# TuringQ/deepquantum

Measured on AMD Instinct MI355X. Metric: gate-applies/sec, 28q random circuit depth 40 (HBM GB/s in roofline), higher is better.
Workload: dtype c64

## Files before the change

### deepquantum_amd/csrc/dq_wave.hip

```cpp
#include <utility>

#include "dq_common.hpp"
#include <stddef.h>
#include <string.h>
#include <stdlib.h>

namespace dq {

#include "dq_wave_asm.inc"
#include "dq_wave_asm64.inc"
#include "dq_wave_valu.inc"
#include "dq_wave_valu64.inc"

constexpr int WAVE_LANES = 6;
constexpr int WAVE_MAX_REC = 112;
constexpr int WAVE_EXT_REC = 256;

struct WaveC64 {
    using real = float;
    using acc_t = float;
    static constexpr int M = 12, R = 6, NA = 64, VB = 1, MAXK = DQ_WAVE_MAXK, ELEM = 8, GRAD_VARIANTS = DQ_WAVE_GRAD_VARIANTS;
    static constexpr unsigned LDS_PER_WAVE = 8448;
    static constexpr int ID_GEN_U = DQ_WID_GEN_U, ID_GEN_C = DQ_WID_GEN_C, ID_GEN_R = DQ_WID_GEN_R, ID_X_U = DQ_WID_X_U,
                         ID_X_C = DQ_WID_X_C, ID_X_R = DQ_WID_X_R, ID_X_R1 = DQ_WID_X_R1, ID_TRIP0 = DQ_WID_TRIP0,
                         ID_DIAG1 = DQ_WID_DIAG1, ID_DIAG2 = DQ_WID_DIAG2, ID_GRAD = DQ_WID_GRAD, ID_EXPZ = DQ_WID_EXPZ, ID_GEN2 = DQ_WID_GEN2, ID_GEN2R = DQ_WID_GEN2R, ID_GEN2X = DQ_WID_GEN2X, ID_GEN2XC = DQ_WID_GEN2XC, ID_SWAP = DQ_WID_SWAP;
    static int trip_id(unsigned mask) { return kWaveTripId[mask]; }
    static int swap_id(int i, int j) { return kWaveSwapId[i][j]; }
    __device__ static __forceinline__ void body(uint64_t kg, uint32_t gend, uint64_t mb, uint32_t moff, uint64_t tg, uint64_t ks,
                                                uint64_t inb, uint64_t outb, uint32_t ldsb, uint32_t tid, uint32_t flags) {
        wave_tile_body_f32(kg, gend, mb, moff, tg, ks, inb, outb, ldsb, tid, flags);
    }
};
struct WaveC128 {
    using real = double;
    using acc_t = double;
    static constexpr int M = 11, R = 5, NA = 32, VB = 0, MAXK = DQ_WAVE64_MAXK, ELEM = 16, GRAD_VARIANTS = DQ_WAVE64_GRAD_VARIANTS;
    static constexpr unsigned LDS_PER_WAVE = 8704;
    static constexpr int ID_GEN_U = DQ_WID64_GEN_U, ID_GEN_C = DQ_WID64_GEN_C, ID_GEN_R = DQ_WID64_GEN_R, ID_X_U = DQ_WID64_X_U,
                         ID_X_C = DQ_WID64_X_C, ID_X_R = DQ_WID64_X_R, ID_X_R1 = DQ_WID64_X_R1, ID_TRIP0 = DQ_WID64_TRIP0,
                         ID_DIAG1 = DQ_WID64_DIAG1, ID_DIAG2 = DQ_WID64_DIAG2, ID_GRAD = DQ_WID64_GRAD, ID_EXPZ = DQ_WID64_EXPZ, ID_GEN2 = DQ_WID64_GEN2, ID_GEN2R = DQ_WID64_GEN2R, ID_GEN2X = -1, ID_GEN2XC = -1, ID_SWAP = DQ_WID64_SWAP;
    static int trip_id(unsigned mask) { return kWave64TripId[mask]; }
    static int swap_id(int i, int j) { return kWave64SwapId[i][j]; }
    __device__ static __forceinline__ void body(uint64_t kg, uint32_t gend, uint64_t mb, uint32_t moff, uint64_t tg, uint64_t ks,
                                                uint64_t inb, uint64_t outb, uint32_t ldsb, uint32_t tid, uint32_t flags) {
        wave_tile_body_f64(kg, gend, mb, moff, tg, ks, inb, outb, ldsb, tid, flags);
    }
};

template <typename T> using vec2 = T __attribute__((ext_vector_type(2)));

struct WaveRec {
    uint32_t w[8];
};

struct WaveKernPass {
    uint64_t load_off[5];
    uint64_t store_off[5];
    uint32_t load_lane_shift[6];
    uint32_t store_lane_shift[6];
    uint32_t tb_contrib[6];
    uint32_t nrec_bytes, mat_base_bytes;
    uint8_t read_blk_pos[DQ_FUSED_MAX_BLK];
    uint8_t store_blk_pos[DQ_FUSED_MAX_BLK];
    uint32_t zext;
    uint32_t fix_read[2], fix_write[2];
    uint32_t reserved[3];
    WaveRec rec[WAVE_MAX_REC];
};
static_assert(offsetof(WaveKernPass, store_off) == 40 && offsetof(WaveKernPass, load_lane_shift) == 80 &&
                  offsetof(WaveKernPass, tb_contrib) == 128 && offsetof(WaveKernPass, zext) == 208 &&
                  offsetof(WaveKernPass, rec) == 240, "descriptor layout");

struct WaveKernArgs {
    const void* in;
    void* out;
    const void* mats;
    int64_t mat_bstride;
    int64_t in_bstride;
    int n;
    int tpw;
    WaveKernPass p;
    double* grads;
    int64_t grad_bstride;
    const void* ext_rec;
};
static_assert(sizeof(WaveKernArgs) <= 4096 && (offsetof(WaveKernArgs, p) + offsetof(WaveKernPass, rec)) % 32 == 0, "kernel-argument segment");

template <class W, bool GRAD>
__global__ __launch_bounds__(256) void wave_pass_kernel(const vec2<typename W::real>* in, vec2<typename W::real>* out,
                                                        const vec2<typename W::real>* mats, int64_t mat_bstride,
                                                        int64_t in_bstride, int n, int tpw_flags, const WaveKernPass p,
                                                        double* grads, int64_t grad_bstride, const void* ext_rec) {
    (void)in, (void)out, (void)mats, (void)mat_bstride;
    extern __shared__ __attribute__((aligned(16))) unsigned char dq_wave_smem[];
    (void)dq_wave_smem;
    const unsigned tid = threadIdx.x;
    if constexpr (GRAD) {
        for (unsigned i = tid; i < p.nrec_bytes / 4u; i += 256u)
            *(__attribute__((address_space(3))) typename W::acc_t*)(uintptr_t)(4u * W::LDS_PER_WAVE + (unsigned)sizeof(typename W::acc_t) * i) = 0;
        __syncthreads();
    }
    const unsigned wave = (unsigned)__builtin_amdgcn_readfirstlane((int)(tid >> 6));
    unsigned grp = blockIdx.x, sample = blockIdx.y;
    if (in_bstride == 0 && (gridDim.x & 7u) == 0) {
        const unsigned lin = blockIdx.y * gridDim.x + blockIdx.x, nb = gridDim.y;
        const unsigned group = lin / (8u * nb), r = lin % (8u * nb);
        sample = r >> 3;
        grp = group * 8u + (r & 7u);
    }
    if (const unsigned xv = ((unsigned)tpw_flags >> 18) & 31u) {
        const unsigned q = blockIdx.x >> 3, j = blockIdx.x & 7u;
        if (xv == 31u) grp = j * (gridDim.x >> 3) + q;
        else grp = ((q >> (xv - 1u)) << (xv + 2u)) + (j << (xv - 1u)) + (q & ((1u << (xv - 1u)) - 1u));
    }
  uint32_t tile32 = grp * 4u + wave;
  for (;;) {
    const uint64_t tile_id = tile32;
    typedef const __attribute__((address_space(4))) uint32_t* KWords;
    uint64_t karg = (uint64_t)__builtin_amdgcn_kernarg_segment_ptr();
    asm volatile("" : "+s"(karg));
    const KWords hw = (KWords)(karg + offsetof(WaveKernArgs, p));
    {
        const uint32_t a_tf0 = ((KWords)karg)[offsetof(WaveKernArgs, tpw) / 4];
        const uint32_t ntiles = 1u << (hw[offsetof(WaveKernPass, zext) / 4] & 63u), lper = 2u + (a_tf0 & 0xffu);
        if (tile32 >= ntiles) break;
        tile32 += ((ntiles + (1u << lper) - 1u) >> lper) * 4u;
    }
    uint64_t tg = 0, tw = 0;
#pragma unroll
    for (int w = 0; w < DQ_FUSED_MAX_BLK / 4; ++w) {
        const uint32_t rw = hw[offsetof(WaveKernPass, read_blk_pos) / 4 + w], sw = hw[offsetof(WaveKernPass, store_blk_pos) / 4 + w];
#pragma unroll
        for (int k = 0; k < 4; ++k) {
            const uint64_t bit = (tile_id >> (4 * w + k)) & 1ull;
            tg |= bit << ((rw >> (8 * k)) & 0x3fu);
            tw |= bit << ((sw >> (8 * k)) & 0x3fu);
        }
    }
    {
        const uint32_t fo = offsetof(WaveKernPass, fix_read) / 4;
        tg |= (uint64_t)hw[fo] | ((uint64_t)hw[fo + 1] << 32);
        tw |= (uint64_t)hw[fo + 2] | ((uint64_t)hw[fo + 3] << 32);
    }
    typedef const __attribute__((address_space(4))) uint64_t* KQuads;
    const KQuads kq = (KQuads)karg;
    const uint64_t a_in = kq[0], a_out = kq[1], a_mats = kq[2], a_mbs = kq[3], a_ibs = kq[4];
    const uint64_t a_ext = kq[offsetof(WaveKernArgs, ext_rec) / 8];
    const uint64_t rec_base = a_ext ? a_ext : karg + offsetof(WaveKernArgs, p) + offsetof(WaveKernPass, rec);
    const uint32_t a_n = ((KWords)karg)[offsetof(WaveKernArgs, n) / 4], a_tf = ((KWords)karg)[offsetof(WaveKernArgs, tpw) / 4];
    constexpr uint64_t ES = W::ELEM;
    const uint64_t inb = a_in + ((uint64_t)sample * a_ibs + tg) * ES;
    const uint64_t outb = a_out + (((uint64_t)sample << a_n) + tw) * ES;
    const uint64_t mb = a_mats + (uint64_t)((int64_t)sample * (int64_t)a_mbs) * ES;
    const unsigned flags = ((a_ibs == 0 ? (a_tf >> 16) & ~1u : a_tf >> 16) & 3u) | (hw[offsetof(WaveKernPass, zext) / 4] & 0x003f3f00u);
    W::body(rec_base, hw[offsetof(WaveKernPass, nrec_bytes) / 4], mb,
            hw[offsetof(WaveKernPass, mat_base_bytes) / 4], tg,
            karg + offsetof(WaveKernArgs, p) + offsetof(WaveKernPass, load_off), inb, outb, wave * W::LDS_PER_WAVE, tid,
            flags);
  }
    if constexpr (GRAD) {
        __syncthreads();
        typedef const __attribute__((address_space(4))) uint32_t* KW;
        const KW rw = ext_rec ? (KW)(uint64_t)ext_rec
                              : (KW)((uint64_t)__builtin_amdgcn_kernarg_segment_ptr() + offsetof(WaveKernArgs, p) + offsetof(WaveKernPass, rec));
        const unsigned nrec = p.nrec_bytes / 32u;
        double* const grow = grads + (uint64_t)sample * (uint64_t)grad_bstride;
        for (unsigned i = tid; i < nrec * 8u; i += 256u) {
            const unsigned id = rw[8u * (i >> 3)];
            if ((id >= (unsigned)W::ID_GRAD && id < (unsigned)W::ID_EXPZ) || (id == (unsigned)W::ID_EXPZ && (i & 7u) == 0u)) {
                const typename W::acc_t v = *(__attribute__((address_space(3))) typename W::acc_t*)(uintptr_t)(4u * W::LDS_PER_WAVE + (unsigned)sizeof(typename W::acc_t) * i);
                atomicAdd(grow + (uint64_t)rw[8u * (i >> 3) + 6] * 8u + (i & 7u), (double)v);
            }
        }
    }
}

namespace {

template <class W>
struct Xlate {
    const DqFusedPass* p;
    WaveKernPass* k;
    int phys[W::R];
    int lanes[WAVE_LANES];
    int nrec = 0;
    WaveRec* recs = nullptr;
    int cap = WAVE_MAX_REC;

    bool push(const WaveRec& r) {
        if (nrec >= cap) return false;
        recs[nrec++] = r;
        return true;
    }
    int slot_of(int tile_bit) const {
        for (int s = 0; s < W::R; ++s)
            if (phys[s] == tile_bit) return s;
        return -1;
    }

    bool trip(unsigned mask, const int* inc_lanes, int kk, const int* want) {
        const int a = 5 - kk, S = 64 + (1 << a);
        int moving[W::R], out_bits[W::R], inc_bits[W::R], stay_lanes[WAVE_LANES], stay_bits[WAVE_LANES], fpos[WAVE_LANES];
        int nm = 0, ns = 0;
        for (int s = 0; s < W::R; ++s)
            if ((mask >> s) & 1u) {
                moving[nm] = s;
                out_bits[nm] = phys[s];
                ++nm;
            }
        for (int i = 0; i < kk; ++i) inc_bits[i] = lanes[inc_lanes[i]];
        for (int b = 0; b < WAVE_LANES; ++b) {
            bool inc = false;
            for (int i = 0; i < kk; ++i) inc = inc || inc_lanes[i] == b;
            if (!inc) {
                stay_lanes[ns] = b;
                stay_bits[ns] = lanes[b];
                ++ns;
            }
        }
        if (kk == 0) {
            for (int t = 0; t < ns; ++t) fpos[t] = t;
        } else {
            for (int t = 0; t < ns; ++t) fpos[t] = t < a ? t : 5;
        }
        uint32_t cw[WAVE_LANES] = {0}, cr[WAVE_LANES] = {0}, tbc[WAVE_LANES] = {0};
        for (int i = 0; i < kk; ++i) cw[inc_lanes[i]] = (unsigned)W::ELEM << (a + i);
        for (int t = 0; t < ns; ++t) cw[stay_lanes[t]] = (unsigned)W::ELEM << fpos[t];
        int nl[WAVE_LANES];
        if (want) {
            for (int b = 0; b < WAVE_LANES; ++b) nl[b] = want[b];
        } else if (kk == 0) {
            for (int b = 0; b < WAVE_LANES; ++b) nl[b] = lanes[b];
        } else {
            for (int b = 0; b < WAVE_LANES; ++b) nl[b] = b < a ? stay_bits[b] : (b < 5 ? out_bits[b - a] : stay_bits[a]);
        }
        for (int b = 0; b < WAVE_LANES; ++b) {
            bool found = false;
            for (int i = 0; i < kk && !found; ++i)
                if (nl[b] == out_bits[i]) {
                    cr[b] = ((unsigned)W::ELEM * (unsigned)S) << i;
                    found = true;
                }
            for (int t = 0; t < ns && !found; ++t)
                if (nl[b] == stay_bits[t]) {
                    cr[b] = (unsigned)W::ELEM << fpos[t];
                    found = true;
                }
            if (!found) return false;
            tbc[b] = 1u << nl[b];
        }
        WaveRec ra{}, rb{};
        ra.w[0] = kk == 0 ? (uint32_t)W::ID_TRIP0 : (uint32_t)W::trip_id(mask);
        ra.w[1] = tbc[0], ra.w[2] = tbc[1], ra.w[3] = tbc[2], ra.w[5] = tbc[3], ra.w[6] = tbc[4], ra.w[7] = tbc[5];
        for (int b = 0; b < WAVE_LANES; ++b) rb.w[b] = cw[b] | (cr[b] << 16);
        for (int i = 0; i < kk; ++i) phys[moving[i]] = inc_bits[i];
        for (int b = 0; b < WAVE_LANES; ++b) lanes[b] = nl[b];
        return push(ra) && push(rb);
    }

    bool go(unsigned slotset, const int* want) {
        for (;;) {
            unsigned mask = 0;
            int inc[WAVE_LANES], ninc = 0, nout = 0;
            for (int s = 0; s < W::R; ++s)
                if (!((slotset >> phys[s]) & 1u)) {
                    mask |= 1u << s;
                    ++nout;
                }
            for (int b = 0; b < WAVE_LANES; ++b)
                if ((slotset >> lanes[b]) & 1u) inc[ninc++] = b;
            if (nout != ninc) return false;
            if (nout == 0) return true;
            int kk = nout;
            if (kk > W::MAXK) kk = nout > 2 * W::MAXK ? W::MAXK : (nout + 1) / 2;
            if (kk < nout) {
                unsigned m2 = 0;
                int c = 0;
                for (int s = 0; s < W::R && c < kk; ++s)
                    if ((mask >> s) & 1u) {
                        m2 |= 1u << s;
                        ++c;
                    }
                mask = m2;
            }
            if (!trip(mask, inc, kk, kk == nout ? want : nullptr)) return false;
        }
    }
};

}

template <class W>
static int wave_translate(const DqFusedPass* p, int n, WaveKernPass* k, uint64_t dead = 0, WaveRec* ext = nullptr, int ext_cap = 0,
                          uint64_t fixm = 0, uint64_t fixv = 0) {
    memset(k, 0, sizeof(*k));
    const int L = p->L, h = p->h;
    auto rpos = [&](int tl) { return tl < L ? tl : (int)p->high_pos[tl - L]; };
    auto wpos = [&](int tl) { return tl < L ? (int)p->store_low_pos[tl] : (int)p->store_high_pos[tl - L]; };
    Xlate<W> x;
    x.p = p;
    x.k = k;
    x.recs = ext ? ext : k->rec;
    x.cap = ext ? ext_cap : WAVE_MAX_REC;
    unsigned slotmask = 0;
    for (int s = 0; s < W::R; ++s) {
        x.phys[s] = p->load_rb[s];
        slotmask |= 1u << p->load_rb[s];
    }
    for (int b = 0, q = 0; b < WAVE_LANES; ++b, ++q) {
        while ((slotmask >> q) & 1u) ++q;
        x.lanes[b] = q;
    }
    {
        uint64_t tilemask = (1ull << L) - 1ull;
        for (int i = 0; i < h; ++i) tilemask |= 1ull << p->high_pos[i];
        int nb = 0;
        uint64_t fix_r = 0, fix_w = 0;
        for (int j = 0, q = 0; j < n - W::M; ++j, ++q) {
            while (q < 64 && ((tilemask >> q) & 1ull)) ++q;
            if ((dead >> q) & 1ull) continue;
            if ((fixm >> q) & 1ull) {
                if ((fixv >> q) & 1ull) {
                    fix_r |= 1ull << q;
                    fix_w |= 1ull << p->store_blk_pos[j];
                }
                continue;
            }
            k->read_blk_pos[nb] = (uint8_t)q;
            k->store_blk_pos[nb] = p->store_blk_pos[j];
            ++nb;
        }
        for (int j = nb; j < DQ_FUSED_MAX_BLK; ++j) k->read_blk_pos[j] = k->store_blk_pos[j] = 63;
        k->zext = (uint32_t)nb;
        k->fix_read[0] = (uint32_t)fix_r, k->fix_read[1] = (uint32_t)(fix_r >> 32);
        k->fix_write[0] = (uint32_t)fix_w, k->fix_write[1] = (uint32_t)(fix_w >> 32);
        static const bool by_store = [] { const char* e = getenv("DQ_WAVE_TILE_ORDER"); return !(e && e[0] == 'r'); }();
        if (by_store)
            for (int i = 1; i < nb; ++i)
                for (int j = i; j > 0 && k->store_blk_pos[j] < k->store_blk_pos[j - 1]; --j) {
                    std::swap(k->store_blk_pos[j], k->store_blk_pos[j - 1]);
                    std::swap(k->read_blk_pos[j], k->read_blk_pos[j - 1]);
                }
    }
    for (int s = W::VB; s < W::R; ++s) {
        k->load_off[s - W::VB] = (uint64_t)W::ELEM << rpos(x.phys[s]);
        if ((dead >> rpos(x.phys[s])) & 1ull) k->zext |= 1u << (8 + s);
    }
    for (int b = 0; b < WAVE_LANES; ++b) {
        k->load_lane_shift[b] = (W::ELEM == 8 ? 3u : 4u) + (uint32_t)rpos(x.lanes[b]);
        k->tb_contrib[b] = 1u << x.lanes[b];
        if ((dead >> rpos(x.lanes[b])) & 1ull) k->zext |= 1u << (16 + b);
    }
    k->mat_base_bytes = p->mat_base * (uint32_t)W::ELEM;

    const char* why = "too many records for one pass (gates + layout changes)";
    for (int r = 0; r < p->nrounds; ++r) {
        const DqFusedRound& rd = p->rounds[r];
        unsigned want = 0;
        for (int s = 0; s < W::R; ++s) want |= 1u << rd.rb[s];
        if (!x.go(want, nullptr)) goto fail;
        for (int gi = rd.gate_begin; gi < rd.gate_end; ++gi) {
            const DqFusedGate& g = p->gates[gi];
            if (g.kind == DQ_FG_GEN2 && W::ID_GEN2 >= 0) {
                const int q1 = x.slot_of(rd.rb[g.q]), q2 = x.slot_of(rd.rb[g.q2]);
                const int a = q1 < q2 ? q1 : q2, b = q1 < q2 ? q2 : q1;
                unsigned pc = 0;
                for (int s = 0; s < W::R; ++s)
                    if ((g.reg_cmask >> s) & 1u) pc |= 1u << x.slot_of(rd.rb[s]);
                WaveRec rec{};
                const int body = g.loc == DQ_MODE_XCPLX && W::ID_GEN2XC >= 0 ? W::ID_GEN2XC
                                 : g.loc == DQ_MODE_XREAL && W::ID_GEN2X >= 0 ? W::ID_GEN2X
                                 : (g.loc == DQ_MODE_REAL || g.loc == DQ_MODE_XREAL) && W::ID_GEN2R >= 0 ? W::ID_GEN2R : W::ID_GEN2;
                rec.w[0] = (uint32_t)(body + (W::swap_id(a, b) - W::ID_SWAP));
                rec.w[1] = g.thr_cmask;
                rec.w[2] = (uint32_t)g.out_cmask, rec.w[3] = (uint32_t)(g.out_cmask >> 32);
                rec.w[4] = g.mat_advance;
                for (int j = 0, i = 0; j < W::NA; ++j) {
                    if (((j >> a) & 1) || ((j >> b) & 1)) continue;
                    if (((unsigned)j & pc) == pc) rec.w[5] |= 1u << i;
                    ++i;
                }
                rec.w[6] = q1 == a ? 1u : 0u;
                if (!x.push(rec)) goto fail;
                continue;
            }
            if (g.kind == DQ_FG_EXPZ) {
                unsigned pm = 0;
                for (int s = 0; s < W::R; ++s)
                    if ((g.reg_cmask >> s) & 1u) pm |= 1u << x.slot_of(rd.rb[s]);
                WaveRec rec{};
                rec.w[0] = (uint32_t)W::ID_EXPZ;
                rec.w[1] = g.thr_cmask;
                rec.w[2] = (uint32_t)g.out_cmask, rec.w[3] = (uint32_t)(g.out_cmask >> 32);
                for (int j = 0; j < W::NA; ++j)
                    if (__builtin_popcount((unsigned)j & pm) & 1) rec.w[j < 32 ? 5 : 7] |= 1u << (j & 31);
                rec.w[6] = g.reserved;
                if (!x.push(rec)) goto fail;
                continue;
            }
            if (g.kind == DQ_FG_GRAD && W::ID_GRAD >= 0) {
                int ps = x.slot_of(rd.rb[g.q2]);
                if (ps != 0) {
                    WaveRec sw{};
                    sw.w[0] = (uint32_t)W::swap_id(0, ps);
                    if (!x.push(sw)) goto fail;
                    const int t_ = x.phys[0];
                    x.phys[0] = x.phys[ps];
                    x.phys[ps] = t_;
                }
                const int q = x.slot_of(rd.rb[g.q]);
                unsigned pc = 0;
                for (int s = 0; s < W::R; ++s)
                    if ((g.reg_cmask >> s) & 1u) pc |= 1u << x.slot_of(rd.rb[s]);
                WaveRec rec{};
                const int variant = (int)g.loc < W::GRAD_VARIANTS ? (int)g.loc : 0;
                rec.w[0] = (uint32_t)(W::ID_GRAD + (W::R - 1) * variant + q - 1);
                rec.w[1] = g.thr_cmask;
                rec.w[2] = (uint32_t)g.out_cmask, rec.w[3] = (uint32_t)(g.out_cmask >> 32);
                for (int j = 0, i = 0; j < W::NA; ++j) {
                    if (((j >> q) & 1) || (j & 1)) continue;
                    if (((unsigned)j & pc) == pc) rec.w[5] |= 1u << i;
                    ++i;
                }
                rec.w[6] = g.reserved;
                if (!x.push(rec)) goto fail;
                continue;
            }
            if (g.kind != DQ_FG_GEN1 && g.kind != DQ_FG_X1 && g.kind != DQ_FG_DIAG1 && g.kind != DQ_FG_DIAG2) {
                set_error("dq_apply_fused: the pass kernel takes dense gates on one or two targets, X and diagonal gates (record %d has kind %d); "
                          "such a gate runs on its own (dq_apply_gate_*)", gi, (int)g.kind);
                return DQ_ERR_UNSUPPORTED;
            }
            unsigned pc = 0;
            int nc = 0, onec = 0;
            for (int s = 0; s < W::R; ++s)
                if ((g.reg_cmask >> s) & 1u) {
                    onec = x.slot_of(rd.rb[s]);
                    pc |= 1u << onec;
                    ++nc;
                }
            const bool ctl = g.thr_cmask != 0 || g.out_cmask != 0;
            WaveRec rec{};
            rec.w[1] = g.thr_cmask;
            rec.w[2] = (uint32_t)g.out_cmask, rec.w[3] = (uint32_t)(g.out_cmask >> 32);
            rec.w[4] = g.mat_advance;
            if (g.kind == DQ_FG_DIAG1 || g.kind == DQ_FG_DIAG2) {
                auto regmask = [&](unsigned must_set, unsigned must_clear) {
                    uint64_t mk = 0;
                    for (unsigned j = 0; j < (unsigned)W::NA; ++j)
                        if ((j & must_set) == must_set && (j & must_clear) == 0) mk |= 1ull << j;
                    return mk;
                };
                auto selector = [&](int loc, int q_) -> uint32_t {
                    return loc == DQ_LOC_THR ? ((1u << 6) | (uint32_t)q_) : loc == DQ_LOC_OUT ? ((2u << 6) | (uint32_t)q_) : 0u;
                };
                auto put = [&](int base, int variant, bool masked, uint32_t selA, uint32_t selB, uint32_t idx0, uint32_t idx1,
                               uint64_t mk, uint32_t advance) {
                    WaveRec r2 = rec;
                    r2.w[0] = (uint32_t)(base + variant + (masked ? W::R + 1 : 0));
                    r2.w[4] = advance;
                    r2.w[5] = selA | (selB << 8) | (idx0 << 16) | (idx1 << 24);
                    r2.w[6] = (uint32_t)mk, r2.w[7] = (uint32_t)(mk >> 32);
                    return x.push(r2);
                };
                const bool masked = nc > 0;
                const uint64_t ctlmask = regmask(pc, 0);
                bool ok;
                if (g.kind == DQ_FG_DIAG1) {
                    if (g.loc == DQ_LOC_REG) ok = put(W::ID_DIAG1, 1 + x.slot_of(rd.rb[g.q]), masked, 0, 0, 0x00, 0x55, ctlmask, 4);
                    else ok = put(W::ID_DIAG1, 0, masked, 0, selector(g.loc, g.q), 0x44, 0, ctlmask, 4);
                } else {
                    const bool r1 = g.loc == DQ_LOC_REG, r2_ = g.loc2 == DQ_LOC_REG;
                    const int p1 = r1 ? x.slot_of(rd.rb[g.q]) : -1, p2 = r2_ ? x.slot_of(rd.rb[g.q2]) : -1;
                    if (r1 && r2_) {
                        ok = put(W::ID_DIAG2, 1 + p2, true, 0, 0, 0x00, 0x55, regmask(pc, 1u << p1), 16) &&
                             put(W::ID_DIAG2, 1 + p2, true, 0, 0, 0xAA, 0xFF, regmask(pc | (1u << p1), 0), 0);
                    } else if (r1) {
                        ok = put(W::ID_DIAG2, 1 + p1, masked, selector(g.loc2, g.q2), 0, 0x10, 0x32, ctlmask, 16);
                    } else if (r2_) {
                        ok = put(W::ID_DIAG2, 1 + p2, masked, selector(g.loc, g.q), 0, 0x20, 0x31, ctlmask, 16);
                    } else {
                        ok = put(W::ID_DIAG2, 0, masked, selector(g.loc, g.q), selector(g.loc2, g.q2), 0xE4, 0, ctlmask, 16);
                    }
                }
                if (!ok) goto fail;
                continue;
            }
            const int q = x.slot_of(rd.rb[g.q]);
            if (nc > 0) {
                uint32_t pm = 0;
                for (int j = 0, i = 0; j < W::NA; ++j) {
                    if ((j >> q) & 1) continue;
                    if (((unsigned)j & pc) == pc) pm |= 1u << i;
                    ++i;
                }
                rec.w[5] = pm;
            }
            if (g.kind == DQ_FG_X1) {
                if (nc == 0) rec.w[0] = (ctl ? W::ID_X_C : W::ID_X_U) + q;
                else if (nc == 1) rec.w[0] = W::ID_X_R1 + (W::R - 1) * q + (onec < q ? onec : onec - 1);
                else rec.w[0] = W::ID_X_R + q;
            } else {
                if (nc > 0) rec.w[0] = W::ID_GEN_R + q;
                else if (ctl) rec.w[0] = W::ID_GEN_C + q;
                else rec.w[0] = W::ID_GEN_U + W::R * g.loc + q;
            }
            if (!x.push(rec)) goto fail;
        }
    }
    {
        unsigned want = 0;
        int want_lanes[WAVE_LANES];
        for (int s = 0; s < W::R; ++s) want |= 1u << p->store_rb[s];
        for (int b = 0; b < WAVE_LANES; ++b) want_lanes[b] = p->store_tb[b];
        if (!x.go(want, want_lanes)) goto fail;
        bool same = true;
        for (int b = 0; b < WAVE_LANES; ++b) same = same && x.lanes[b] == want_lanes[b];
        if (!same && !x.trip(0, nullptr, 0, want_lanes)) goto fail;
        const int s0 = W::VB ? x.slot_of(p->store_rb[0]) : 0;
        if (s0 != 0) {
            WaveRec rec{};
            rec.w[0] = (uint32_t)W::swap_id(0, s0);
            if (!x.push(rec)) goto fail;
            const int t = x.phys[0];
            x.phys[0] = x.phys[s0];
            x.phys[s0] = t;
        }
    }
    for (int s = W::VB; s < W::R; ++s) k->store_off[s - W::VB] = (uint64_t)W::ELEM << wpos(x.phys[s]);
    for (int b = 0; b < WAVE_LANES; ++b) k->store_lane_shift[b] = (W::ELEM == 8 ? 3u : 4u) + (uint32_t)wpos(x.lanes[b]);
    k->nrec_bytes = 32u * (unsigned)x.nrec;
    return DQ_OK;
fail:
    set_error("dq_apply_fused (wave tile): %s", why);
    return DQ_ERR_UNSUPPORTED;
}

template <class W, bool GRAD = false>
static int wave_launch(const void* in, void* out, const void* mats, int64_t mat_bstride, int64_t in_bstride, int n, int64_t batch,
                       const DqFusedPass* pass, hipStream_t s, double* grads = nullptr, int64_t ngrads = 0, uint64_t dead = 0,
                       const void* ext_rec = nullptr, int64_t ext_bytes = 0, uint64_t fixm = 0, uint64_t fixv = 0) {
    WaveKernPass kp;
    int rc;
    if (ext_rec) {
        static thread_local WaveRec scratch[WAVE_EXT_REC];
        rc = wave_translate<W>(pass, n, &kp, dead, scratch, WAVE_EXT_REC);
        if (!rc && (int64_t)kp.nrec_bytes != ext_bytes) {
            set_error("dq_apply_fused_grad_ext: %lld bytes of records in device memory, this pass has %u", (long long)ext_bytes, kp.nrec_bytes);
            return DQ_ERR_ARG;
        }
    } else {
        rc = wave_translate<W>(pass, n, &kp, dead, nullptr, 0, fixm, fixv);
    }
    if (rc) return rc;
    const uint64_t tiles = 1ull << (kp.zext & 63u);
    int tpw = 1;
    if (GRAD) {
        static const int gcap = [] { const char* e = getenv("DQ_WAVE_GRAD_TPW"); return e ? atoi(e) : 2; }();
        static const int zcap = [] { const char* e = getenv("DQ_WAVE_EXPZ_TPW"); return e ? atoi(e) : 2; }();
        bool only_expz = !ext_rec;
        for (unsigned r = 0; only_expz && r < kp.nrec_bytes / 32u; ++r)
            only_expz = !(kp.rec[r].w[0] >= (uint32_t)W::ID_GRAD && kp.rec[r].w[0] < (uint32_t)W::ID_EXPZ);
        const int cap = only_expz ? zcap : gcap;
        while (tpw < cap && (tiles * (uint64_t)batch) / (8ull * (uint64_t)tpw) >= 2048) tpw *= 2;
    } else {
        static const int tpw_env = [] { const char* e = getenv("DQ_WAVE_TPW"); return e ? atoi(e) : 1; }();
        while (tpw < tpw_env && (tiles * (uint64_t)batch) / (8ull * (uint64_t)tpw) >= 2048) tpw *= 2;
    }
    dim3 grid((unsigned)((tiles + 4ull * tpw - 1) / (4ull * tpw)), (unsigned)batch);
    const size_t acc_rec = ext_rec ? (size_t)kp.nrec_bytes / 32u : (size_t)WAVE_MAX_REC;
    size_t lds = 4 * W::LDS_PER_WAVE + (GRAD ? acc_rec * 8 * sizeof(typename W::acc_t) : 0);
    if (const char* kb = getenv("DQ_WAVE_LDS_KB")) {
        lds = (size_t)atoi(kb) << 10;
        hipFuncSetAttribute(reinterpret_cast<const void*>(&wave_pass_kernel<W, GRAD>), hipFuncAttributeMaxDynamicSharedMemorySize, (int)lds);
    }
    static const int nt_env = [] { const char* e = getenv("DQ_WAVE_NT"); return e ? atoi(e) & 3 : -1; }();
    const uint64_t state_bytes = ((uint64_t)batch << n) * (uint64_t)W::ELEM;
    const int nt = nt_env >= 0 ? nt_env : (state_bytes >= (1ull << 30) ? 3 : 0);
    static const int xcd_env = [] { const char* e = getenv("DQ_WAVE_XCD"); return e ? atoi(e) : 1; }();
    int xcd = 0;
    static const int xcd_tpw = [] { const char* e = getenv("DQ_WAVE_XCD_TPW"); return e ? atoi(e) : 1; }();
    if (xcd_env && in_bstride != 0 && (tpw == 1 || xcd_tpw)) {
        if (xcd_env == 1 && (grid.x & 7u) == 0) xcd = 31;
        else if (xcd_env > 1 && (xcd_env & (xcd_env - 1)) == 0 && grid.x % (8u * (unsigned)xcd_env) == 0)
            xcd = 32 - __builtin_clz((unsigned)xcd_env);
    }
    using V = vec2<typename W::real>;
    hipLaunchKernelGGL((wave_pass_kernel<W, GRAD>), grid, dim3(256), lds, s, static_cast<const V*>(in), static_cast<V*>(out),
                       static_cast<const V*>(mats), mat_bstride, in_bstride, n, (31 - __builtin_clz((unsigned)tpw)) | (nt << 16) | (xcd << 18), kp, grads, ngrads * 8,
                       ext_rec);
    return check_launch("dq_apply_fused (wave tile)");
}

int wave_launch_c64(const void* in, void* out, const void* mats, int64_t mat_bstride, int64_t in_bstride, int n, int64_t batch,
                    const DqFusedPass* pass, hipStream_t s, uint64_t dead, uint64_t fixm, uint64_t fixv) {
    return wave_launch<WaveC64>(in, out, mats, mat_bstride, in_bstride, n, batch, pass, s, nullptr, 0, dead, nullptr, 0, fixm, fixv);
}
int wave_launch_grad_c64(const void* in, void* out, const void* mats, int64_t mat_bstride, int64_t in_bstride, int n, int64_t batch,
                         const DqFusedPass* pass, hipStream_t s, double* grads, int64_t ngrads, const void* ext_rec, int64_t ext_bytes) {
    return wave_launch<WaveC64, true>(in, out, mats, mat_bstride, in_bstride, n, batch, pass, s, grads, ngrads, 0, ext_rec, ext_bytes);
}
int wave_launch_grad_c128(const void* in, void* out, const void* mats, int64_t mat_bstride, int64_t in_bstride, int n, int64_t batch,
                          const DqFusedPass* pass, hipStream_t s, double* grads, int64_t ngrads, const void* ext_rec, int64_t ext_bytes) {
    return wave_launch<WaveC128, true>(in, out, mats, mat_bstride, in_bstride, n, batch, pass, s, grads, ngrads, 0, ext_rec, ext_bytes);
}
int wave_launch_c128(const void* in, void* out, const void* mats, int64_t mat_bstride, int64_t in_bstride, int n, int64_t batch,
                     const DqFusedPass* pass, hipStream_t s, uint64_t dead, uint64_t fixm, uint64_t fixv) {
    return wave_launch<WaveC128>(in, out, mats, mat_bstride, in_bstride, n, batch, pass, s, nullptr, 0, dead, nullptr, 0, fixm, fixv);
}

}

extern "C" int64_t dq_wave_records(const DqFusedPass* pass, int n, void* out, int64_t max_bytes) {
    if (!pass) {
        dq::set_error("dq_wave_records: null pointer");
        return DQ_ERR_ARG;
    }
    static thread_local dq::WaveRec scratch[dq::WAVE_EXT_REC];
    dq::WaveKernPass kp;
    int rc;
    if (pass->m == 12 && pass->slots == 6) rc = dq::wave_translate<dq::WaveC64>(pass, n, &kp, 0, scratch, dq::WAVE_EXT_REC);
    else if (pass->m == 11 && pass->slots == 5) rc = dq::wave_translate<dq::WaveC128>(pass, n, &kp, 0, scratch, dq::WAVE_EXT_REC);
    else {
        dq::set_error("dq_wave_records: not a wave-tile pass (m = %d, %d slots)", pass->m, pass->slots);
        return DQ_ERR_ARG;
    }
    if (rc) return rc;
    const int64_t bytes = kp.nrec_bytes;
    if (out && max_bytes > 0) memcpy(out, scratch, (size_t)(bytes < max_bytes ? bytes : max_bytes));
    return bytes;
}

extern "C" int dq_wave_descriptor(const DqFusedPass* pass, int n, uint64_t known_zero, void* out, int max_bytes) {
    if (!pass) {
        dq::set_error("dq_wave_descriptor: null pointer");
        return DQ_ERR_ARG;
    }
    static thread_local dq::WaveRec scratch[dq::WAVE_EXT_REC];
    dq::WaveKernPass kp;
    int rc;
    if (pass->m == 12 && pass->slots == 6) rc = dq::wave_translate<dq::WaveC64>(pass, n, &kp, known_zero, scratch, dq::WAVE_EXT_REC);
    else if (pass->m == 11 && pass->slots == 5) rc = dq::wave_translate<dq::WaveC128>(pass, n, &kp, known_zero, scratch, dq::WAVE_EXT_REC);
    else {
        dq::set_error("dq_wave_descriptor: not a wave-tile pass (m = %d, %d slots)", pass->m, pass->slots);
        return DQ_ERR_ARG;
    }
    if (rc) return rc;
    const int head = (int)offsetof(dq::WaveKernPass, rec);
    const int bytes = head + (int)kp.nrec_bytes;
    if (out && max_bytes > 0) {
        memcpy(out, &kp, head < max_bytes ? head : max_bytes);
        if (max_bytes > head) memcpy((char*)out + head, scratch, (size_t)((bytes < max_bytes ? bytes : max_bytes) - head));
    }
    return bytes;
}

namespace dq {
template <class W>
static int wave_pass_cost(const DqFusedPass* pass, int n, uint64_t known_zero, const unsigned short* table, int nids,
                          int64_t* valu, double* bytes_moved) {
    static thread_local WaveRec scratch[WAVE_EXT_REC];
    WaveKernPass kp;
    const int rc = wave_translate<W>(pass, n, &kp, known_zero, scratch, WAVE_EXT_REC);
    if (rc) return rc;
    int64_t v = 0;
    const unsigned nrec = kp.nrec_bytes / 32u;
    for (unsigned r = 0; r < nrec; ++r) {
        const uint32_t id = scratch[r].w[0];
        if (id < (uint32_t)nids) v += table[id];
        if (id >= (uint32_t)W::ID_TRIP0 && id < (uint32_t)W::ID_SWAP) ++r;
    }
    if (valu) *valu = v;
    if (bytes_moved) {
        const double nt = (double)(1ull << (kp.zext & 63u));
        const int unloaded = __builtin_popcount((kp.zext >> 8) & 0x3f3fu);
        *bytes_moved = nt * (double)W::ELEM * ((double)(1u << W::M) + (double)((1u << W::M) >> unloaded));
    }
    return DQ_OK;
}
}

extern "C" int dq_wave_pass_cost(const DqFusedPass* pass, int n, uint64_t known_zero, int64_t* valu, double* bytes_moved) {
    if (!pass) {
        dq::set_error("dq_wave_pass_cost: null pointer");
        return DQ_ERR_ARG;
    }
    if (pass->m == 12 && pass->slots == 6)
        return dq::wave_pass_cost<dq::WaveC64>(pass, n, known_zero, dq::kWaveValu, DQ_WAVE_NIDS, valu, bytes_moved);
    if (pass->m == 11 && pass->slots == 5)
        return dq::wave_pass_cost<dq::WaveC128>(pass, n, known_zero, dq::kWave64Valu, DQ_WAVE64_NIDS, valu, bytes_moved);
    dq::set_error("dq_wave_pass_cost: not a wave-tile pass (m = %d, %d slots)", pass->m, pass->slots);
    return DQ_ERR_ARG;
}

extern "C" int dq_wave_handler_valu(int c128, int id) {
    if (id < 0 || id >= (c128 ? DQ_WAVE64_NIDS : DQ_WAVE_NIDS)) return -1;
    return c128 ? dq::kWave64Valu[id] : dq::kWaveValu[id];
}

namespace dq {
template <class W>
static int wave_gate_valu(const unsigned short* table, int opclass) {
    const int q = W::R / 2;
    switch (opclass) {
        case 0: return 0;
        case 1: case 2: case 3: case 4: return table[W::ID_GEN_U + W::R * (opclass - 1) + q];
        case 5: return table[W::ID_GEN_C + q];
        case 6: return table[W::ID_X_U + q];
        case 7: return (table[W::ID_X_C + q] + table[W::ID_X_R1 + (W::R - 1) * q]) / 2;
        case 8: return table[W::trip_id((1u << W::MAXK) - 1u)];
        default: return -1;
    }
}
}

extern "C" int dq_wave_gate_valu(int c128, int opclass) {
    return c128 ? dq::wave_gate_valu<dq::WaveC128>(dq::kWave64Valu, opclass) : dq::wave_gate_valu<dq::WaveC64>(dq::kWaveValu, opclass);
}
```

Before: 87790.

## Search LDS transpose placements to minimize bank conflicts in wave layout changes

After: 88360, median of 6. About the same (+0.6%).

```diff
diff --git a/deepquantum_amd/csrc/dq_wave.hip b/deepquantum_amd/csrc/dq_wave.hip
--- a/deepquantum_amd/csrc/dq_wave.hip
+++ b/deepquantum_amd/csrc/dq_wave.hip
@@ -1,3 +1,5 @@
+#include <algorithm>
+#include <unordered_map>
 #include <utility>
 
 #include "dq_common.hpp"
@@ -177,12 +179,118 @@
 
 namespace {
 
+struct TripPlace {
+    uint8_t sigma[4];
+    uint8_t fz[WAVE_LANES];
+    uint8_t src[WAVE_LANES];
+    uint16_t cost;
+};
+constexpr int TRIP_SWAP_EST = 4;
+
+template <class W>
+static int trip_write_extra(const uint32_t* c) {
+    constexpr int GL = W::ELEM == 8 ? 16 : 8, MOD = W::ELEM == 8 ? 16 : 8;
+    int cnt[16] = {0}, worst = 0;
+    for (int l = 0; l < GL; ++l) {
+        uint32_t ad = 0;
+        for (int b = 0; b < 4; ++b)
+            if ((l >> b) & 1) ad += c[b];
+        const int v = ++cnt[ad % MOD];
+        worst = v > worst ? v : worst;
+    }
+    return (64 / GL) * (worst - 1);
+}
+template <class W>
+static int trip_read_extra(const uint32_t* c) {
+    constexpr int MOD = W::ELEM == 8 ? 32 : 16;
+    int cnt[2][32] = {{0}}, worst[2] = {1, 1};
+    for (int l = 0; l < 32; ++l) {
+        uint32_t ad = 0;
+        for (int b = 0; b < 5; ++b)
+            if ((l >> b) & 1) ad += c[b];
+        const int g = W::ELEM == 8 ? 0 : ((l >> 2) ^ (l >> 3) ^ (l >> 4)) & 1;
+        const int v = ++cnt[g][ad % MOD];
+        worst[g] = v > worst[g] ? v : worst[g];
+    }
+    return 2 * ((worst[0] - 1) + (worst[1] - 1));
+}
+
+template <class W>
+static const TripPlace& trip_solve(int kk, unsigned incmask, const uint8_t* wantsrc, unsigned nextmask, int pref_pos, int pref_inc) {
+    static thread_local std::unordered_map<uint64_t, TripPlace> memo;
+    uint64_t key = (uint64_t)kk | ((uint64_t)incmask << 3) | ((uint64_t)(wantsrc != nullptr) << 9) | ((uint64_t)nextmask << 34) |
+                   ((uint64_t)(pref_pos + 1) << 44) | ((uint64_t)(pref_inc + 1) << 47);
+    if (wantsrc)
+        for (int b = 0; b < WAVE_LANES; ++b) key |= (uint64_t)wantsrc[b] << (10 + 4 * b);
+    {
+        const auto it = memo.find(key);
+        if (it != memo.end()) return it->second;
+    }
+    const int a = 5 - kk, ns = WAVE_LANES - kk, S = 64 + (1 << a);
+    int inc[WAVE_LANES], stay[WAVE_LANES], ni = 0, nst = 0;
+    for (int b = 0; b < WAVE_LANES; ++b) ((incmask >> b) & 1u ? inc[ni++] : stay[nst++]) = b;
+    TripPlace best{};
+    best.cost = 0xffff;
+    int sig[4] = {0, 1, 2, 3};
+    do {
+        const int pen = pref_pos >= 0 && sig[pref_pos] != pref_inc ? TRIP_SWAP_EST : 0;
+        for (int ti = ns - 1; ti >= 0 && best.cost; --ti) {
+            {
+                int low[WAVE_LANES], nlow = 0;
+                for (int t = 0; t < ns; ++t)
+                    if (t != ti) low[nlow++] = t;
+                do {
+                    uint8_t fz[WAVE_LANES] = {0};
+                    uint32_t cw[WAVE_LANES] = {0}, sc[16] = {0};
+                    for (int j = 0; j < nlow; ++j) fz[low[j]] = (uint8_t)(1 << j);
+                    fz[ti] = 32;
+                    for (int i = 0; i < kk; ++i) cw[inc[sig[i]]] = 1u << (a + i), sc[i] = (uint32_t)S << i;
+                    for (int t = 0; t < ns; ++t) cw[stay[t]] = fz[t], sc[8 + t] = fz[t];
+                    const int wc = trip_write_extra<W>(cw) + pen;
+                    if (wc >= best.cost) continue;
+                    auto consider = [&](const uint8_t* src) {
+                        uint32_t cr[WAVE_LANES];
+                        for (int b = 0; b < WAVE_LANES; ++b) cr[b] = sc[src[b]];
+                        int tot = wc + trip_read_extra<W>(cr);
+                        if (tot >= best.cost) return;
+                        if (nextmask) {
+                            unsigned nm = 0;
+                            for (int b = 0; b < WAVE_LANES; ++b)
+                                if ((nextmask >> (src[b] < 8 ? src[b] : 4 + src[b] - 8)) & 1u) nm |= 1u << b;
+                            tot += trip_solve<W>(__builtin_popcount(nm), nm, nullptr, 0, -1, -1).cost;
+                            if (tot >= best.cost) return;
+                        }
+                        best.cost = (uint16_t)tot;
+                        for (int i = 0; i < 4; ++i) best.sigma[i] = (uint8_t)sig[i];
+                        for (int t = 0; t < WAVE_LANES; ++t) best.fz[t] = fz[t], best.src[t] = src[t];
+                    };
+                    if (wantsrc) {
+                        consider(wantsrc);
+                    } else {
+                        uint8_t src[WAVE_LANES];
+                        for (int j = 0; j < nlow; ++j) src[j] = (uint8_t)(8 + low[j]);
+                        for (int i = 0; i < kk; ++i) src[a + i] = (uint8_t)i;
+                        src[5] = (uint8_t)(8 + ti);
+                        consider(src);
+                        std::sort(src, src + WAVE_LANES);
+                        do consider(src);
+                        while (best.cost && std::next_permutation(src, src + WAVE_LANES));
+                    }
+                } while (best.cost && std::next_permutation(low, low + nlow));
+            }
+        }
+    } while (best.cost && std::next_permutation(sig, sig + kk));
+    return memo.emplace(key, best).first->second;
+}
+
 template <class W>
 struct Xlate {
     const DqFusedPass* p;
     WaveKernPass* k;
     int phys[W::R];
     int lanes[WAVE_LANES];
+    int pref0 = -1;
+    int cost = 0;
     int nrec = 0;
     WaveRec* recs = nullptr;
     int cap = WAVE_MAX_REC;
@@ -198,55 +306,59 @@
         return -1;
     }
 
-    bool trip(unsigned mask, const int* inc_lanes, int kk, const int* want) {
+    bool trip(unsigned mask, const int* inc_lanes, int kk, const int* want, unsigned next_inc = 0) {
         const int a = 5 - kk, S = 64 + (1 << a);
-        int moving[W::R], out_bits[W::R], inc_bits[W::R], stay_lanes[WAVE_LANES], stay_bits[WAVE_LANES], fpos[WAVE_LANES];
+        int moving[W::R], out_bits[W::R], stay_lanes[WAVE_LANES], stay_bits[WAVE_LANES];
         int nm = 0, ns = 0;
+        unsigned incmask = 0;
         for (int s = 0; s < W::R; ++s)
             if ((mask >> s) & 1u) {
                 moving[nm] = s;
                 out_bits[nm] = phys[s];
                 ++nm;
             }
-        for (int i = 0; i < kk; ++i) inc_bits[i] = lanes[inc_lanes[i]];
-        for (int b = 0; b < WAVE_LANES; ++b) {
-            bool inc = false;
-            for (int i = 0; i < kk; ++i) inc = inc || inc_lanes[i] == b;
-            if (!inc) {
+        for (int i = 0; i < kk; ++i) incmask |= 1u << inc_lanes[i];
+        for (int b = 0; b < WAVE_LANES; ++b)
+            if (!((incmask >> b) & 1u)) {
                 stay_lanes[ns] = b;
                 stay_bits[ns] = lanes[b];
                 ++ns;
             }
-        }
-        if (kk == 0) {
-            for (int t = 0; t < ns; ++t) fpos[t] = t;
-        } else {
-            for (int t = 0; t < ns; ++t) fpos[t] = t < a ? t : 5;
-        }
+        uint8_t wantsrc[WAVE_LANES];
+        if (want)
+            for (int b = 0; b < WAVE_LANES; ++b) {
+                int src = -1;
+                for (int i = 0; i < kk; ++i)
+                    if (want[b] == out_bits[i]) src = i;
+                for (int t = 0; t < ns; ++t)
+                    if (want[b] == stay_bits[t]) src = 8 + t;
+                if (src < 0) return false;
+                wantsrc[b] = (uint8_t)src;
+            }
+        unsigned nextmask = 0;
+        for (int i = 0; i < kk; ++i)
+            if ((next_inc >> out_bits[i]) & 1u) nextmask |= 1u << i;
+        for (int t = 0; t < ns; ++t)
+            if ((next_inc >> stay_bits[t]) & 1u) nextmask |= 16u << t;
+        if (__builtin_popcount(nextmask) > W::MAXK) nextmask = 0;
+        int pref_pos = -1, pref_inc = -1;
+        if (pref0 >= 0 && kk > 0 && (mask & 1u))
+            for (int i = 0; i < kk; ++i)
+                if (lanes[inc_lanes[i]] == pref0) pref_pos = 0, pref_inc = i;
+        const TripPlace& pl = trip_solve<W>(kk, incmask, want ? wantsrc : nullptr, nextmask, pref_pos, pref_inc);
+        cost += pl.cost;
         uint32_t cw[WAVE_LANES] = {0}, cr[WAVE_LANES] = {0}, tbc[WAVE_LANES] = {0};
-        for (int i = 0; i < kk; ++i) cw[inc_lanes[i]] = (unsigned)W::ELEM << (a + i);
-        for (int t = 0; t < ns; ++t) cw[stay_lanes[t]] = (unsigned)W::ELEM << fpos[t];
-        int nl[WAVE_LANES];
-        if (want) {
-            for (int b = 0; b < WAVE_LANES; ++b) nl[b] = want[b];
-        } else if (kk == 0) {
-            for (int b = 0; b < WAVE_LANES; ++b) nl[b] = lanes[b];
-        } else {
-            for (int b = 0; b < WAVE_LANES; ++b) nl[b] = b < a ? stay_bits[b] : (b < 5 ? out_bits[b - a] : stay_bits[a]);
-        }
+        int inc_bits[W::R], nl[WAVE_LANES];
+        for (int i = 0; i < kk; ++i) {
+            const int lane = inc_lanes[pl.sigma[i]];
+            cw[lane] = (unsigned)W::ELEM << (a + i);
+            inc_bits[i] = lanes[lane];
+        }
+        for (int t = 0; t < ns; ++t) cw[stay_lanes[t]] = (unsigned)W::ELEM * pl.fz[t];
         for (int b = 0; b < WAVE_LANES; ++b) {
-            bool found = false;
-            for (int i = 0; i < kk && !found; ++i)
-                if (nl[b] == out_bits[i]) {
-                    cr[b] = ((unsigned)W::ELEM * (unsigned)S) << i;
-                    found = true;
-                }
-            for (int t = 0; t < ns && !found; ++t)
-                if (nl[b] == stay_bits[t]) {
-                    cr[b] = (unsigned)W::ELEM << fpos[t];
-                    found = true;
-                }
-            if (!found) return false;
+            const int src = pl.src[b];
+            nl[b] = src < 8 ? out_bits[src] : stay_bits[src - 8];
+            cr[b] = src < 8 ? ((unsigned)W::ELEM * (unsigned)S) << src : (unsigned)W::ELEM * pl.fz[src - 8];
             tbc[b] = 1u << nl[b];
         }
         WaveRec ra{}, rb{};
@@ -258,7 +370,7 @@
         return push(ra) && push(rb);
     }
 
-    bool go(unsigned slotset, const int* want) {
+    bool go(unsigned slotset, const int* want, unsigned nextset = 0) {
         for (;;) {
             unsigned mask = 0;
             int inc[WAVE_LANES], ninc = 0, nout = 0;
@@ -272,6 +384,7 @@
             if (nout != ninc) return false;
             if (nout == 0) return true;
             int kk = nout;
+            unsigned rest = 0;
             if (kk > W::MAXK) kk = nout > 2 * W::MAXK ? W::MAXK : (nout + 1) / 2;
             if (kk < nout) {
                 unsigned m2 = 0;
@@ -282,8 +395,22 @@
                         ++c;
                     }
                 mask = m2;
-            }
-            if (!trip(mask, inc, kk, kk == nout ? want : nullptr)) return false;
+                unsigned all = 0, bestsub = 0;
+                int bestcost = 1 << 30;
+                for (int i = 0; i < ninc; ++i) all |= 1u << inc[i];
+                for (unsigned sub = 1; sub < 64u; ++sub) {
+                    if ((sub & ~all) || __builtin_popcount(sub) != kk) continue;
+                    const int c2 = trip_solve<W>(kk, sub, nullptr, 0, -1, -1).cost;
+                    if (c2 < bestcost) bestcost = c2, bestsub = sub;
+                }
+                ninc = 0;
+                for (int b = 0; b < WAVE_LANES; ++b) {
+                    if ((bestsub >> b) & 1u) inc[ninc++] = b;
+                    else if ((all >> b) & 1u) rest |= 1u << lanes[b];
+                }
+            }
+            const bool last = kk == nout;
+            if (!trip(mask, inc, kk, last ? want : nullptr, last ? (nextset ? nextset & ~slotset : 0u) : rest)) return false;
         }
     }
 };
@@ -302,6 +429,7 @@
     x.k = k;
     x.recs = ext ? ext : k->rec;
     x.cap = ext ? ext_cap : WAVE_MAX_REC;
+    x.pref0 = W::VB ? (int)p->store_rb[0] : -1;
     unsigned slotmask = 0;
     for (int s = 0; s < W::R; ++s) {
         x.phys[s] = p->load_rb[s];
@@ -310,6 +438,27 @@
     for (int b = 0, q = 0; b < WAVE_LANES; ++b, ++q) {
         while ((slotmask >> q) & 1u) ++q;
         x.lanes[b] = q;
+    }
+    static const int kTop3[6][3] = {{3, 4, 5}, {3, 5, 4}, {4, 3, 5}, {4, 5, 3}, {5, 3, 4}, {5, 4, 3}};
+    int r1 = 0;
+    auto round_slots = [&](int r) {
+        unsigned m = 0;
+        for (int s = 0; s < W::R; ++s) m |= 1u << (r < p->nrounds ? p->rounds[r].rb[s] : p->store_rb[s]);
+        return m;
+    };
+    while (r1 < p->nrounds && round_slots(r1) == slotmask) ++r1;
+    if (r1 < p->nrounds) {
+        const unsigned first = round_slots(r1), second = round_slots(r1 + 1);
+        int best = 0, bestcost = 1 << 30;
+        WaveRec tmp[16];
+        for (int c = 0; c < 6; ++c) {
+            Xlate<W> y = x;
+            y.recs = tmp, y.cap = 16, y.nrec = 0;
+            for (int j = 0; j < 3; ++j) y.lanes[3 + j] = x.lanes[kTop3[c][j]];
+            if (y.go(first, nullptr, second) && y.cost < bestcost) best = c, bestcost = y.cost;
+        }
+        const int l3[3] = {x.lanes[kTop3[best][0]], x.lanes[kTop3[best][1]], x.lanes[kTop3[best][2]]};
+        for (int j = 0; j < 3; ++j) x.lanes[3 + j] = l3[j];
     }
     {
         uint64_t tilemask = (1ull << L) - 1ull;
@@ -358,7 +507,9 @@
         const DqFusedRound& rd = p->rounds[r];
         unsigned want = 0;
         for (int s = 0; s < W::R; ++s) want |= 1u << rd.rb[s];
-        if (!x.go(want, nullptr)) goto fail;
+        unsigned after = 0;
+        for (int s = 0; s < W::R; ++s) after |= 1u << (r + 1 < p->nrounds ? p->rounds[r + 1].rb[s] : p->store_rb[s]);
+        if (!x.go(want, nullptr, after)) goto fail;
         for (int gi = rd.gate_begin; gi < rd.gate_end; ++gi) {
             const DqFusedGate& g = p->gates[gi];
             if (g.kind == DQ_FG_GEN2 && W::ID_GEN2 >= 0) {
@@ -513,6 +664,25 @@
         int want_lanes[WAVE_LANES];
         for (int s = 0; s < W::R; ++s) want |= 1u << p->store_rb[s];
         for (int b = 0; b < WAVE_LANES; ++b) want_lanes[b] = p->store_tb[b];
+        {
+            int best = 0, bestcost = 1 << 30;
+            WaveRec tmp[16];
+            for (int c = 0; c < 6; ++c) {
+                Xlate<W> y = x;
+                y.recs = tmp, y.cap = 16, y.nrec = 0, y.cost = 0;
+                int wl[WAVE_LANES];
+                for (int b = 0; b < WAVE_LANES; ++b) wl[b] = b < 3 ? want_lanes[b] : want_lanes[kTop3[c][b - 3]];
+                if (!y.go(want, wl)) continue;
+                bool same = true;
+                for (int b = 0; b < WAVE_LANES; ++b) same = same && y.lanes[b] == wl[b];
+                if (!same && !y.trip(0, nullptr, 0, wl)) continue;
+                if (W::VB && y.slot_of(p->store_rb[0]) != 0) y.cost += TRIP_SWAP_EST;
+                if (!same) y.cost += 1;
+                if (y.cost < bestcost) best = c, bestcost = y.cost;
+            }
+            const int l3[3] = {want_lanes[kTop3[best][0]], want_lanes[kTop3[best][1]], want_lanes[kTop3[best][2]]};
+            for (int j = 0; j < 3; ++j) want_lanes[3 + j] = l3[j];
+        }
         if (!x.go(want, want_lanes)) goto fail;
         bool same = true;
         for (int b = 0; b < WAVE_LANES; ++b) same = same && x.lanes[b] == want_lanes[b];
```
